# jfjell/Octree-Raymarcher

Measured on AMD Instinct MI355X. Metric: Mrays/s (primary+shadow) at 1920x1080, depth-12 SVO, higher is better.
Workload: dtype f32; 1 GPU; c3_1080p_depth12_4x1x4_shadow; depth_per_chunk=12, chunksize=128, nodes=99473656, bricks=34206642, hbm_pool_bytes=11087035656, kernel=auto, launches_in_flight=2, frames_per_launch=16, frames_in_flight=32, gather=False, partition=single, ranks_seen=1, launcher=single process

## Files before the change

octree-raymarcher_amd/csrc/kernel_stack.hip.h:

```cpp
#pragma once
#include "march.hip.h"
#include "step_asm.hip.h"
#include "chunk_step_asm.hip.h"

namespace svo {

constexpr int CW_ESCAPE_PENDING = (int)0x80000000;
enum : int { M_DONE = 0, M_WORLD = 1, M_HIT = 2, M_TREE = 3, M_TWIG = 4 };

constexpr int VOTE_WORLD = 8;
constexpr int VOTE_HIT = 16;
constexpr int VOTE_BUSY = 24;
constexpr int CREEP_SERIOUS = 6;
constexpr int CREEP_LANES = 8;
#define SVO_LIKELY(x) __builtin_expect(!!(x), 1)
#define SVO_UNLIKELY(x) __builtin_expect(!!(x), 0)
constexpr int STEP_EXTRA = 4;
constexpr int STEP_LANES = 8;
constexpr int DRAIN_STEPS = 8;
#ifndef SVO_SURE_MISS_WHEN
#define SVO_SURE_MISS_WHEN __builtin_amdgcn_readfirstlane(more ? 0 : 1)
#endif

__device__ __forceinline__ float recip_pow2(float x) { return __uint_as_float(0x7F000000u - __float_as_uint(x)); }

__device__ __forceinline__ unsigned long long vote(bool p) { return __builtin_amdgcn_ballot_w64(p); }
__device__ __forceinline__ int vote_count(unsigned long long m)
{
    int n = (int)__popcll(m);
    asm("" : "+s"(n));
    return n;
}

struct ChunkGrid {
    float inv;
    int32_t off[3];
    int32_t dimw, dimh, dimd;
    uint32_t table_in_lds;
};
static_assert(sizeof(ChunkGrid) == 32, "two 16-byte LDS reads");

__device__ __forceinline__ int wrap_once(int m, int dim)
{
    const uint32_t a = (uint32_t)m, b = (uint32_t)(m + dim), c = (uint32_t)(m - dim);
    return (int)min(min(a, b), c);
}

__device__ __forceinline__ void chunk_cell_pow2(const ChunkGrid &G, V3 p, int &mx, int &my, int &mz)
{
    float qx = p.x * G.inv, qy = p.y * G.inv, qz = p.z * G.inv;
    if (qx < 0.0f) qx -= 1.0f;
    if (qy < 0.0f) qy -= 1.0f;
    if (qz < 0.0f) qz -= 1.0f;
    const int ix = (int)qx, iy = (int)qy, iz = (int)qz;
    mx = wrap_once(ix + G.off[0], G.dimw); my = wrap_once(iy + G.off[1], G.dimh); mz = wrap_once(iz + G.off[2], G.dimd);
}
__device__ __forceinline__ uint32_t mad_u24(uint32_t a, uint32_t b, uint32_t c)
{
    uint32_t r;
    asm("v_mad_u32_u24 %0, %1, %2, %3" : "=v"(r) : "v"(a), "v"(b), "v"(c));
    return r;
}
__device__ __forceinline__ int chunk_index_u24(const ChunkGrid &G, int mx, int my, int mz)
{
    return (int)mad_u24(mad_u24((uint32_t)my, (uint32_t)G.dimd, (uint32_t)mz), (uint32_t)G.dimw, (uint32_t)mx);
}

__device__ __forceinline__ V3 cube_normal_pow2(V3 s, V3 lo, float size, float eps)
{
    const V3 hi = lo + size;
    const V3 c = (lo + hi) * 0.5f;
    const V3 p = s - c;
    const float d = fabsf(lo.x - hi.x) * 0.5f;
    const float invd = recip_pow2(d);
    const float b = 1.0f + eps;
    const float ix = (float)(int)((p.x * invd) * b), iy = (float)(int)((p.y * invd) * b), iz = (float)(int)((p.z * invd) * b);
    const float dot = ix * ix + iy * iy + iz * iz;
    float inv;
    if (dot == 1.0f) inv = 1.0f;
    else if (dot == 2.0f) inv = __uint_as_float(0x3F3504F3u);
    else if (dot == 3.0f) inv = __uint_as_float(0x3F13CD3Au);
    else inv = 1.0f / sqrtf(dot);
    return mk(ix * inv, iy * inv, iz * inv);
}

__device__ __forceinline__ uint32_t child_slot(int ux, int uy, int uz, int sh)
{
    const uint32_t bx = __builtin_amdgcn_ubfe((uint32_t)ux, (uint32_t)sh, 1u);
    const uint32_t by = __builtin_amdgcn_ubfe((uint32_t)uy, (uint32_t)sh, 1u);
    const uint32_t bz = __builtin_amdgcn_ubfe((uint32_t)uz, (uint32_t)sh, 1u);
    return ((bz << 1) + by) * 2u + bx;
}
__device__ __forceinline__ uint32_t ld_node(const uint32_t *pool, uint32_t boff)
{
    return *reinterpret_cast<const uint32_t *>(reinterpret_cast<const char *>(pool) + (size_t)boff);
}
constexpr uint32_t WIDE_PAYLOAD = (1u << 25) - 1u;
__device__ __forceinline__ uint32_t wide_slot(int ux, int uy, int uz, int sh)
{
    const uint32_t bx = __builtin_amdgcn_ubfe((uint32_t)ux, (uint32_t)sh, 2u);
    const uint32_t by = __builtin_amdgcn_ubfe((uint32_t)uy, (uint32_t)sh, 2u);
    const uint32_t bz = __builtin_amdgcn_ubfe((uint32_t)uz, (uint32_t)sh, 2u);
    return (bz << 4) | (by << 2) | bx;
}
__device__ __forceinline__ bool is_branch(uint32_t word) { return (int32_t)word < (int32_t)0xC0000000; }

__device__ __forceinline__ TraceArgs args_reloaded()
{
    auto p = __builtin_amdgcn_kernarg_segment_ptr();
    asm volatile("" : "+s"(p));
    TraceArgs T;
    __builtin_memcpy(&T, p, sizeof T);
    return T;
}
__device__ __forceinline__ FrameCam camera_reloaded(int f)
{
    auto p = __builtin_amdgcn_kernarg_segment_ptr();
    asm volatile("" : "+s"(p));
    FrameCam c;
    __builtin_memcpy(&c, (decltype(p))((const char __attribute__((address_space(4))) *)p + __builtin_offsetof(TraceArgs, cams) + (size_t)f * sizeof(FrameCam)), sizeof c);
    return c;
}

__device__ __noinline__ float brick_layer_first_touch(int k, V3 a, V3 b, V3 g, V3 bmin, float r, unsigned long long mask)
{
    const float ak = k == 0 ? a.x : k == 1 ? a.y : a.z, bk = k == 0 ? b.x : k == 1 ? b.y : b.z, mk_ = k == 0 ? bmin.x : k == 1 ? bmin.y : bmin.z;
    const float au = k == 0 ? a.y : k == 1 ? a.z : a.x, av = k == 0 ? a.z : k == 1 ? a.x : a.y;
    const float gu = k == 0 ? g.y : k == 1 ? g.z : g.x, gv = k == 0 ? g.z : k == 1 ? g.x : g.y;
    const float mu = k == 0 ? bmin.y : k == 1 ? bmin.z : bmin.x, mv = k == 0 ? bmin.z : k == 1 ? bmin.x : bmin.y;
    const int su = k == 0 ? 4 : k == 1 ? 16 : 1, sv = k == 0 ? 16 : k == 1 ? 1 : 4;
    const float delta = r * 0.0625f;
    bool ok = (ak == mk_) & (bk < 0.0f);
    ok &= (mu >= 4.0f * r) & (mv >= 4.0f * r) & (delta >= (fabsf(mu) + fabsf(mv) + 8.0f * r) * 0x1p-21f);
    ok = ok && fabsf(gu) < 1.0e30f && fabsf(gv) < 1.0e30f;
    if (!ok) return -1.0f;
    const float u0 = au - mu, v0 = av - mv;
    float first = __uint_as_float(0x7F800000u);
    bool clean = true;
    for (int cv = 0; cv < 4; ++cv) {
        const float va = ((float)cv * r - delta - v0) * gv, vb = ((float)(cv + 1) * r + delta - v0) * gv;
        const float v_in = fminf(va, vb), v_out = fmaxf(va, vb);
        for (int cu = 0; cu < 4; ++cu) {
            const bool occupied = (mask >> (cu * su + cv * sv)) & 1ull;
            const float ua = ((float)cu * r - delta - u0) * gu, ub = ((float)(cu + 1) * r + delta - u0) * gu;
            const float s_in = fmaxf(fmaxf(fminf(ua, ub), v_in), 0.0f), s_out = fminf(fmaxf(ua, ub), v_out);
            clean &= (s_in == s_in) & (s_out == s_out);
            first = (occupied & (s_in <= s_out)) ? fminf(first, s_in) : first;
        }
    }
    return clean ? first * (1.0f - 0x1p-18f) : -1.0f;
}

__device__ __forceinline__ void note_tile_cost(int outk, uint32_t steps)
{
    const TraceArgs T = args_reloaded();
    if (!T.tile_cost) return;
    const int k = outk & 0x7FFFFFFF;
    int tile, frame = 0;
    if (T.from_camera) {
        const int per = T.w * T.h;
        frame = k / per;
        const int r = k - frame * per;
        const int ly = r / T.w, lx = r - ly * T.w;
        tile = (ly / TILE_H) * T.tiles_per_row + lx / TILE_W;
    } else tile = k >> 6;
    atomicMax(&T.tile_cost[((size_t)frame * (size_t)T.ntiles + (size_t)tile) * 2 + (outk < 0 ? 1 : 0)], steps);
}

template <bool GLSL>
__device__ __forceinline__ bool past_far_end(int mode, float t, float tt_saved, float tw, float eps, float far)
{
    const float tt = mode == M_TWIG ? tt_saved : t;
    return (mode == M_TREE || mode == M_TWIG) && tw + (GLSL ? tt : tt - eps) >= far;
}

template <int MAXLV, int REFILL, int WAVES_PER_SIMD, bool BIG, bool GLSL, bool SEG = false>
__global__ __launch_bounds__(64, WAVES_PER_SIMD) void k_trace_stack(TraceArgs A)
{
    __shared__ uint32_t stk[MAXLV / 2 + 1][64];
    __shared__ float tile_ray[SEG ? 12 : 11][64];
    constexpr int CHUNK_TAB = (BIG && MAXLV <= 10) ? 126 : MAXLV > 16 ? 62 : 64;
    __shared__ uint32_t chunk_tab[6][CHUNK_TAB];
    __shared__ __attribute__((aligned(16))) ChunkGrid chunk_grid;
    stk[0][threadIdx.x] = 0u;
    const int lane = threadIdx.x;
    const bool want_cost = A.tile_cost != nullptr;
    [[maybe_unused]] const bool light_clear = (A.light_clear & LIGHT_CLEAR_NODES) != 0;
    const int n_chunks = A.dimw * A.dimh * A.dimd;
    const bool chunks_in_lds = n_chunks <= CHUNK_TAB;
    if (lane == 0) {
        chunk_grid.inv = A.inv_chunksize;
        for (int a = 0; a < 3; ++a) chunk_grid.off[a] = A.cbase[a] - A.ccm[a];
        chunk_grid.dimw = A.dimw; chunk_grid.dimh = A.dimh; chunk_grid.dimd = A.dimd;
        chunk_grid.table_in_lds = chunks_in_lds ? 1u : 0u;
    }
    if (chunks_in_lds)
        for (int i = lane; i < n_chunks; i += 64) {
            const DevWide ch = A.wchunks[i];
            chunk_tab[0][i] = __float_as_uint(ch.bmin[0]); chunk_tab[1][i] = __float_as_uint(ch.bmin[1]); chunk_tab[2][i] = __float_as_uint(ch.bmin[2]);
            chunk_tab[3][i] = ch.levels; chunk_tab[4][i] = ch.wide_off; chunk_tab[5][i] = (uint32_t)ch.twig_off;
        }
    __syncthreads();
#ifdef SVO_STACK_TIMING
    const unsigned long long t_begin = __builtin_amdgcn_s_memrealtime();
    unsigned n_iters = 0, n_tree_lanes = 0, n_twig_lanes = 0, n_world_lanes = 0;
    unsigned n_world_runs = 0, n_hit_runs = 0, n_refill = 0, n_tilegen = 0, n_fix = 0;
    unsigned n_lane_twig = 0;
    unsigned n_lane_busy = 0;
    unsigned n_creep_runs = 0, n_creep_rounds = 0, n_dbg = 0;
    unsigned n_wsteps = 0, n_lsteps = 0, n_hit_wait = 0, n_dead_wait = 0, n_wsteps_b = 0, n_lsteps_b = 0, n_world_wait = 0, n_twig_b = 0;
#endif
    [[maybe_unused]] StepStats step_stats;

    const V3 wlo = ld3(A.worldmin), whi = ld3(A.worldmax);
    const V3 sdir = ld3(A.sdir);
    const V3 sg = recip(sdir);
    const float eps = A.eps;
    const bool eps_pow2 = (__float_as_uint(eps) & 0x807FFFFFu) == 0u && __float_as_uint(eps) >= 0x00800000u && __float_as_uint(eps) < 0x7F800000u;
    const float csize = A.chunksize;

    const int tr_cols = A.tiles_per_row;
    const int tr_rows = A.ntiles / (tr_cols > 0 ? tr_cols : 1);
    const bool by_cols = tr_cols >= TILE_REGIONS;
    const int reg_q = (by_cols ? tr_cols : tr_rows) / TILE_REGIONS, reg_rem = (by_cols ? tr_cols : tr_rows) % TILE_REGIONS;
    int region = (int)(__builtin_amdgcn_s_getreg(20 | (0 << 6) | (3 << 11)) & (TILE_REGIONS - 1));
    int regions_left = TILE_REGIONS;
    int tile_first = 0;
    int tile_next = 64;
    bool more = true;
    unsigned rays_marched = 0;

    int mode = M_DONE;
    int outk = 0;
    V3 alpha = mk(0, 0, 0), beta = mk(0, 0, 1), g = mk(0, 0, 0);
    float tw = 0.0f;
    [[maybe_unused]] float far = __uint_as_float(0x7F800000u);
    int cw = 0;
    uint32_t guard = 0;
    V3 O = mk(0, 0, 0), Blo = mk(0, 0, 0);
    float res = 1.0f, t = 0.0f;
    int cnt = 0;
    float tt_saved = 0.0f, t_miss = 0.0f;
    int it_saved = 0;
    V3 clo = mk(0, 0, 0);
    WideRef<BIG> wide_b = 0;
    auto ld_wide = [&](uint32_t e) -> uint32_t {
        if constexpr (BIG) return *reinterpret_cast<const uint32_t *>((size_t)wide_b + ((size_t)e << 2));
        else return ld_node(A.wide, wide_b + (e << 2));
    };
    uint32_t twig_off = 0;
    int levels = 0, ci = -1;
    int pux = 0, puy = 0, puz = 0, valid = 0, plev = 0;
    unsigned long long bmask = 0;
#ifndef SVO_CXX_STEP
    float bsize = 0.0f, res_tree = 1.0f;
    int nw_chunk = 1;
    const uint32_t lds_lane = (uint32_t)(size_t)(__attribute__((address_space(3))) uint32_t *)&stk[0][lane];
    StepUniform SU;
    SU.csize = csize; SU.eps = eps; SU.eps2 = 2.0f * eps; SU.cap_twig = A.cap_twig; SU.wide = A.wide; SU.mask = A.mask; SU.descend_shift = MAXLV <= 10 ? DESCEND_SHIFT_SHALLOW : DESCEND_SHIFT_DEEP;
    const uint32_t lds_tab = (uint32_t)(size_t)(__attribute__((address_space(3))) uint32_t *)&chunk_tab[0][0];
    ChunkStepUniform CU;
    CU.wlo = wlo; CU.whi = whi; CU.csize = csize; CU.eps = eps; CU.cap_chunk = A.cap_chunk; CU.cap_tree = A.cap_tree; CU.wide = A.wide;
    CU.kernarg = __builtin_amdgcn_kernarg_segment_ptr();
#endif
    int creepn = 0;
    for (;;) {
        unsigned long long dead = vote(mode == M_DONE);
        while (more && vote_count(dead) >= REFILL) {
            if (tile_next >= 64) {
                int t32 = -1, tcol = 0, trow = 0, tframe = 0;
                const uint32_t *order = args_reloaded().tile_order;
                if (order) {
                    regions_left = 0;
                    unsigned long long tix = 0;
                    if (lane == 0) tix = atomicAdd(&A.work[WORK_CURSOR0], 1ull);
                    int t = __builtin_amdgcn_readfirstlane((int)tix);
                    if (t < A.ntiles * A.nframes) {
                        tframe = t / A.ntiles; t -= tframe * A.ntiles;
                        t32 = (int)order[t];
                        if ((uint32_t)t32 >= (uint32_t)A.ntiles) { t32 = 0; tframe = -1; }
                        trow = t32 / tr_cols; tcol = t32 - trow * tr_cols;
                    }
                }
                while (regions_left > 0) {
                    const int span = reg_q + (region < reg_rem ? 1 : 0);
                    const int first = region * reg_q + (region < reg_rem ? region : reg_rem);
                    const int count = span * (by_cols ? tr_rows : tr_cols);
                    unsigned long long tix = 0;
                    if (lane == 0) tix = atomicAdd(&A.work[WORK_CURSOR0 + region], 1ull);
                    int t = __builtin_amdgcn_readfirstlane((int)tix);
                    if (t < count * A.nframes) {
                        if (A.nframes > 1) { tframe = t / count; t -= tframe * count; }
                        if (by_cols) { trow = t / span; tcol = first + (t - trow * span); }
                        else { trow = first + t / tr_cols; tcol = t % tr_cols; }
                        t32 = trow * tr_cols + tcol;
                        break;
                    }
                    region = (region + 1) & (TILE_REGIONS - 1);
                    --regions_left;
                }
                if (t32 < 0) { more = false; break; }
                tile_first = t32 * 64;
                tile_next = 0;
#ifdef SVO_STACK_TIMING
                ++n_tilegen;
#endif
                {
                    const TraceArgs T = args_reloaded();
                    const int id = tile_first + lane;
                    bool ok;
                    int k = -1;
                    V3 o = mk(0, 0, 0), d = mk(0, 0, 1);
                    if (T.from_camera) {
                        const int lx = tcol * TILE_W + (lane & (TILE_W - 1));
                        const int ly = trow * TILE_H + lane / TILE_W;
                        ok = (lx < T.w) & (ly < T.h) & (tframe >= 0);
                        k = (tframe * T.h + ly) * T.w + lx;
                        int px = 0, py = 0;
                        if (ok) local_to_pixel(T, lx, ly, px, py);
                        if (ok && (py >= T.imgh || px >= T.imgw)) { store_miss(A.out, k, 0); ok = false; }
                        if (ok) camera_ray(camera_reloaded(tframe), T.imgw, T.imgh, px, py, o, d);
                    } else {
                        ok = id < T.n && tframe >= 0;
                        k = id;
                        if (ok) { o = ld3(T.origins + 3 * (long long)id); d = ld3(T.dirs + 3 * (long long)id); }
                        if constexpr (SEG) tile_ray[11][lane] = ok ? T.tmax[id] : 0.0f;
                    }
                    const V3 gg = recip(d);
                    float t0 = 0.0f;
                    if (ok) {
                        bool hit = true;
                        if (!inside(o, wlo, whi)) t0 = (GLSL ? enter_glsl(o, gg, wlo, whi, hit) : enter(o, d, wlo, whi, hit)) + eps;
                        rays_marched++;
                        if (!hit) { store_miss(A.out, k, 0); ok = false; }
                    }
                    tile_ray[0][lane] = o.x; tile_ray[1][lane] = o.y; tile_ray[2][lane] = o.z;
                    tile_ray[3][lane] = d.x; tile_ray[4][lane] = d.y; tile_ray[5][lane] = d.z;
                    tile_ray[6][lane] = gg.x; tile_ray[7][lane] = gg.y; tile_ray[8][lane] = gg.z;
                    tile_ray[9][lane] = t0;
                    tile_ray[10][lane] = __int_as_float(ok ? k : -1);
                    __syncthreads();
                }
            }
#ifdef SVO_STACK_TIMING
            ++n_refill;
#endif
            const int rank = (int)__builtin_amdgcn_mbcnt_hi((unsigned)(dead >> 32), __builtin_amdgcn_mbcnt_lo((unsigned)dead, 0u));
            const int avail = 64 - tile_next;
            if (mode == M_DONE && rank < avail) {
                const int slot = tile_next + rank;
                const int k = __float_as_int(tile_ray[10][slot]);
                if (k >= 0) {
                    outk = k;
                    alpha = mk(tile_ray[0][slot], tile_ray[1][slot], tile_ray[2][slot]);
                    beta = mk(tile_ray[3][slot], tile_ray[4][slot], tile_ray[5][slot]);
                    g = mk(tile_ray[6][slot], tile_ray[7][slot], tile_ray[8][slot]);
                    tw = tile_ray[9][slot];
                    if constexpr (SEG) far = tile_ray[11][slot];
                    cw = 0; guard = 0; creepn = 0;
                    mode = M_WORLD;
                }
            }
            const int ndead = vote_count(dead);
            tile_next += (ndead < avail) ? ndead : avail;
            __syncthreads();
            dead = vote(mode == M_DONE);
        }
        if (dead == ~0ull) break;
#ifdef SVO_STACK_TIMING
        ++n_iters;
        n_tree_lanes += __popcll(__ballot(mode == M_TREE)); n_twig_lanes += __popcll(__ballot(mode == M_TWIG));
        n_world_lanes += __popcll(__ballot(mode == M_WORLD));
#endif

        const int n_busy = vote_count(vote(mode == M_TREE || mode == M_TWIG));
        const int n_world = vote_count(vote(mode == M_WORLD));
        const int n_hit = vote_count(vote(mode == M_HIT));
        const bool few_busy = n_busy < VOTE_BUSY;
        bool run_world = n_world >= (few_busy ? 1 : VOTE_WORLD);
        if (!run_world && n_world > 0) run_world = vote(mode == M_WORLD && creepn <= -CREEP_SERIOUS) != 0ull;
        const bool run_hit = n_hit >= (few_busy ? 1 : VOTE_HIT);

        if (SVO_UNLIKELY(mode != M_DONE && mode != M_HIT && ++guard > STEP_GUARD)) {
            if (outk < 0) store_flags(A.out, outk & 0x7FFFFFFF, SVO_HIT_FLAG | SVO_SHADOW_TRACED | SVO_ERR_FLAG | (A.normal_mode == SVO_NORMAL_FACE ? (uint32_t)SVO_FACE_NORMAL : 0u));
            else store_miss(A.out, outk, SVO_ERR_FLAG);
            mode = M_DONE;
        }

#ifdef SVO_STACK_TIMING
        n_world_runs += run_world; n_hit_runs += run_hit;
#endif
        if (SVO_LIKELY(run_world)) { asm volatile("");
#ifndef SVO_CXX_STEP
        const ChunkGrid G = chunk_grid;
        const unsigned long long missed = ChunkStepAsm<BIG, GLSL, SEG>::template run<CHUNK_TAB>(
            mode, tw, cw, ci, valid, pux, puy, puz, clo, wide_b, twig_off, levels, O, t, cnt, Blo, res, bsize, res_tree, nw_chunk,
            alpha, beta, g, far, G.inv, G.off[0], G.off[1], G.off[2], G.dimw, G.dimh, G.dimd,
            (uint32_t)__builtin_amdgcn_readfirstlane((int)G.table_in_lds), lds_tab, CU);
        if (__builtin_amdgcn_inverse_ballot_w64(missed)) {
            int k = outk;
            asm("" : "+v"(k));
            if (k >= 0) store_miss(A.out, k, 0);
            if (want_cost) note_tile_cost(k, guard);
            mode = M_DONE;
        }
#else
        if (mode == M_WORLD) {
            if (cw < 0) {
                cw &= ~CW_ESCAPE_PENDING;
                if constexpr (GLSL) tw += guarded(escape(O, g, clo, clo + csize), eps) + eps;
                else tw += escape(O, g, clo, clo + csize) + eps;
            }
            bool miss = cw >= A.cap_chunk;
            if constexpr (SEG) miss |= (GLSL ? tw : tw - eps) >= far;
            if (!miss) {
                cw++;
// ... 44 lines not shown
        }

        int pass = 0;
        const int fixed_steps = (n_busy >= STEP_LANES && vote(creepn > 0 || creepn <= -4 * CREEP_SERIOUS) == 0ull) ? STEP_EXTRA : 0;
#ifndef SVO_CXX_STEP
        const unsigned long long shadow_lanes = light_clear ? vote(outk < 0) : 0ull;
#endif
        for (;;) {
#ifdef SVO_STACK_TIMING
        n_lane_twig += mode == M_TWIG ? (pass == 0 ? 1u + (unsigned)fixed_steps : (unsigned)DRAIN_STEPS) : 0u;
        n_lane_busy += (mode == M_TREE || mode == M_TWIG) ? (pass == 0 ? 1u + (unsigned)fixed_steps : (unsigned)DRAIN_STEPS) : 0u;
        { const int nm = __popcll(__ballot(mode == M_TREE || mode == M_TWIG)); n_wsteps += nm > 0; n_lsteps += nm; if (more) { n_wsteps_b += nm > 0; n_lsteps_b += nm; n_hit_wait += __popcll(__ballot(mode == M_HIT)); n_dead_wait += __popcll(__ballot(mode == M_DONE)); n_world_wait += __popcll(__ballot(mode == M_WORLD)); n_twig_b += __popcll(__ballot(mode == M_TWIG)); } }
#endif
#ifndef SVO_CXX_STEP
        const int nsteps = pass == 0 ? 1 + fixed_steps : DRAIN_STEPS;
        const int sure_miss = SVO_SURE_MISS_WHEN;
        march_steps_asm<BIG, GLSL>(mode, O, Blo, bsize, res, t, cnt, tt_saved, t_miss, it_saved, tw, cw, pux, puy, puz, valid, plev, bmask, creepn,
                                   beta, g, clo, alpha, levels, nw_chunk, res_tree, wide_b, twig_off, lds_lane, SU, nsteps | (sure_miss << 16), shadow_lanes, step_stats);
        pass += nsteps - 1;
#else
        if (mode == M_TREE || mode == M_TWIG) {
            enum : int { S_LEAVE = 0, S_ADVANCE = 1, S_ENTER = 2, S_HIT_LEAF = 3, S_HIT_CELL = 4, S_BAD = 5 };
            const bool twig = mode == M_TWIG;
            const float Bsize = twig ? res * 4.0f : csize, inv_res = recip_pow2(res);
            const int crept = creepn < 0 ? -creepn : creepn;
            creepn = -crept;
            bool leave = cnt <= 0;
            cnt -= 1;
            const V3 p = O + beta * t;
            leave |= !inside(p, Blo, Blo + Bsize);
            const float fx = (p.x - Blo.x) * inv_res, fy = (p.y - Blo.y) * inv_res, fz = (p.z - Blo.z) * inv_res;
            int ux = (int)fx, uy = (int)fy, uz = (int)fz;
#ifdef SVO_STACK_TIMING
            n_fix += __ballot(!twig && ((fx == (float)ux) | (fy == (float)uy) | (fz == (float)uz))) != 0;
#endif
            if (SVO_UNLIKELY(!twig && ((fx == (float)ux) | (fy == (float)uy) | (fz == (float)uz)))) {
                const int nmax = (1 << levels) - 1;
                ux = ux > nmax ? nmax : ux; uy = uy > nmax ? nmax : uy; uz = uz > nmax ? nmax : uz;
                ux -= (Blo.x + (float)ux * res > p.x) ? 1 : 0;
                uy -= (Blo.y + (float)uy * res > p.y) ? 1 : 0;
                uz -= (Blo.z + (float)uz * res > p.z) ? 1 : 0;
            }
            if (twig) leave |= (ux > 3) | (uy > 3) | (uz > 3);

            int what = S_LEAVE;
            int low = 0;
            uint32_t payload = 0;
            if (SVO_LIKELY(!leave)) {
                if (!twig) {
                    const uint32_t diff = (uint32_t)((ux ^ pux) | (uy ^ puy) | (uz ^ puz));
                    const int nw = levels ? (levels + 1) >> 1 : 1;
                    const int hb = 32 - __clz((int)(diff | 1u));
                    const int keep = nw - ((hb + 1) >> 1);
                    int k;
                    asm("v_med3_i32 %0, %1, 0, %2" : "=v"(k) : "v"(keep), "v"(valid));
                    uint32_t wnode = stk[k][lane];
                    int sh = 2 * (nw - 1 - k);
                    uint32_t word = ld_wide((wnode << 6) + wide_slot(ux, uy, uz, sh));
                    while (is_branch(word)) {
                        wnode = word & WIDE_PAYLOAD;
                        ++k;
                        stk[k][lane] = wnode;
                        sh -= 2;
                        word = ld_wide((wnode << 6) + wide_slot(ux, uy, uz, sh));
                    }
                    valid = k; pux = ux; puy = uy; puz = uz;
                    plev = (int)((word >> 25) & 31u);
                    low = (1 << (levels - plev)) - 1;
                    const uint32_t type = node_type(word);
                    what = type == EMPTY ? S_ADVANCE : type == LEAF ? S_HIT_LEAF : S_ENTER;
                    payload = word;
                } else {
                    payload = (uint32_t)(uz * 16 + uy * 4 + ux);
                    what = ((bmask >> payload) & 1ull) ? S_HIT_CELL : S_ADVANCE;
                }
            }

            if (what == S_ADVANCE || what == S_ENTER) {
                const V3 E_lo = mk(Blo.x + (float)(ux & ~low) * res, Blo.y + (float)(uy & ~low) * res, Blo.z + (float)(uz & ~low) * res);
                const float E_size = res * (float)(low + 1);
                const float e = (GLSL ? guarded(escape(p, g, E_lo, E_lo + E_size), eps) : escape(p, g, E_lo, E_lo + E_size)) + eps;
                if (what == S_ADVANCE) {
                    t += e;
                    creepn = e < 2.0f * eps ? crept + 1 : 0;
                } else {
                    bmask = A.mask[twig_off + (payload & WIDE_PAYLOAD)];
                    tt_saved = t; t_miss = t + e; it_saved = cnt;
                    O = p; t = 0.0f; cnt = A.cap_twig;
                    Blo = E_lo;
                    res = E_size * 0.25f;
                    mode = M_TWIG;
                }
            }
            if (leave) {
                if (twig) {
                    t = t_miss;
                    cnt = it_saved;
                    O = alpha + beta * tw;
                    Blo = clo;
                    res = csize * __uint_as_float((uint32_t)(127 - levels) << 23);
                    mode = M_TREE;
                } else {
                    cw |= CW_ESCAPE_PENDING;
                    mode = M_WORLD;
                }
            }
            if (what == S_HIT_LEAF) {
                tw = tw + (GLSL ? t : t - eps);
                cnt = (int)SVO_CELL_NONE;
                mode = M_HIT;
            }
            if (what == S_HIT_CELL) {
                float sdist = t;
                sdist += tt_saved;
                tw = tw + sdist;
                cnt = (int)payload;
                mode = M_HIT;
            }
        }
#endif

        ++pass;
        if (pass <= fixed_steps) continue;
        if (more || pass >= 256) break;
        const unsigned long long marching = vote(mode == M_TREE || mode == M_TWIG);
        if (marching == 0ull || marching != vote(mode != M_DONE) || vote(creepn > 0 || creepn <= -4 * CREEP_SERIOUS) != 0ull) break;
        if constexpr (SEG) if (vote(past_far_end<GLSL>(mode, t, tt_saved, tw, eps, far)) != 0ull) break;
        }
        guard += pass - 1;
        if constexpr (SEG) {
            if (past_far_end<GLSL>(mode, t, tt_saved, tw, eps, far)) {
                if (mode == M_TWIG) O = alpha + beta * tw;
                creepn = creepn > 0 ? -creepn : creepn;
                cw |= CW_ESCAPE_PENDING;
                mode = M_WORLD;
            }
        }

#include "creep_block.inc"

        if (mode == M_HIT && outk < 0) {
            store_flags(A.out, outk & 0x7FFFFFFF, SVO_HIT_FLAG | SVO_SHADOW_TRACED | SVO_SHADOWED | (A.normal_mode == SVO_NORMAL_FACE ? (uint32_t)SVO_FACE_NORMAL : 0u));
            if (want_cost) note_tile_cost(outk, guard);
            mode = M_DONE;
        }
        if constexpr (SEG) {
            if (mode == M_HIT && !(tw < far)) {
                store_miss(A.out, outk, 0);
                if (want_cost) note_tile_cost(outk, guard);
                mode = M_DONE;
            }
        }
        if (run_hit) { asm volatile("");
        if (mode == M_HIT) {
            const int nw = levels ? (levels + 1) >> 1 : 1;
            const uint32_t wn = valid > 0 ? stk[valid][lane] : 0u, slot = wide_slot(pux, puy, puz, 2 * (nw - 1 - valid));
            const uint32_t word = ld_wide((wn << 6) + slot);
            uint32_t node = 0u;
            if (plev != 0) {
                const uint32_t ci = ((slot >> 1) & 1u) | ((slot >> 2) & 2u) | ((slot >> 3) & 4u);
                const uint32_t gi = (slot & 1u) | ((slot >> 1) & 2u) | ((slot >> 2) & 4u);
                size_t wnode_in_pool;
                if constexpr (BIG) wnode_in_pool = (((size_t)wide_b - (size_t)A.wide) >> 8) + wn;
                else wnode_in_pool = (wide_b >> 8) + wn;
                const uint32_t *wb = A.wbase + wnode_in_pool * WIDE_BASE_WORDS;
                const int level_child = 2 * valid + 1 - (2 * nw - levels);
                const bool child = plev == level_child;
                node = wb[child ? 0u : 1u + ci] + (child ? ci : gi);
            }
            const uint32_t hitc = (uint32_t)cnt;
            V3 vlo;
            float vsize;
            uint32_t material;
            if (hitc == SVO_CELL_NONE) {
                const int low = (1 << (levels - plev)) - 1;
                vlo = mk(Blo.x + (float)(pux & ~low) * res, Blo.y + (float)(puy & ~low) * res, Blo.z + (float)(puz & ~low) * res);
                vsize = res * (float)(low + 1);
                material = word & 0xFFFFu;
            } else {
                vlo = mk(Blo.x + (float)(hitc & 3u) * res, Blo.y + (float)((hitc >> 2) & 3u) * res, Blo.z + (float)(hitc >> 4) * res);
                vsize = res;
                const unsigned long long brick = (unsigned long long)twig_off + (word & WIDE_PAYLOAD);
                const uint32_t bw = A.bmat[brick];
                material = bw == BMAT_SEVERAL ? A.twig[brick * TWIG_WORDS + hitc] : (bw & BMAT_MATERIAL_MASK) | ((bw & BMAT_CLEAR_BIT) << 1);
            }
            const V3 point = alpha + beta * (tw - eps);
            uint32_t dark = 0u;
            if constexpr (!GLSL && !SEG) {
                const uint32_t use = (uint32_t)A.light_clear & (uint32_t)(LIGHT_CLEAR_BRICKS | LIGHT_CLEAR_DARK);
                if (use != 0u) {
                    const float inv_res = recip_pow2(res);
                    const float dx = point.x - Blo.x, dy = point.y - Blo.y, dz = point.z - Blo.z;
                    const uint32_t ux = (uint32_t)(int)(dx * inv_res), uy = (uint32_t)(int)(dy * inv_res), uz = (uint32_t)(int)(dz * inv_res);
                    const bool located = (hitc != SVO_CELL_NONE) & (dx >= 0.0f) & (dy >= 0.0f) & (dz >= 0.0f) & ((ux | uy | uz) <= 3u);
                    const uint32_t occupied = (uint32_t)(bmask >> ((uz * 16u + uy * 4u + ux) & 63u)) & 1u;
                    const uint32_t on = (use >> (1u + occupied)) & (occupied | (material >> 16)) & 1u;
                    const uint32_t settle = located ? on : 0u;
                    material = (material & 0xFFFFu) | (settle << 16);
                    dark = (settle & occupied) * (uint32_t)SVO_SHADOWED;
                } else {
                    material &= 0xFFFFu;
                }
            }
            const bool face = A.normal_mode == SVO_NORMAL_FACE;
            const V3 n = face ? face_normal(point, vlo, vlo + vsize, beta) : cube_normal_pow2(point, vlo, vsize, eps);
            const uint32_t flags = SVO_HIT_FLAG | (A.shadow ? SVO_SHADOW_TRACED : 0u) | (face ? (uint32_t)SVO_FACE_NORMAL : 0u) | dark;
            store_hit(A.out, outk, tw, n, material, flags, (uint32_t)ci, node, hitc);
            if (want_cost) note_tile_cost(outk, guard);
            mode = M_DONE;
            if (A.shadow) {
                alpha = point; beta = sdir; g = sg;
                outk |= (int)0x80000000;
                if constexpr (SEG) far = __uint_as_float(0x7F800000u);
                tw = 0.0f; cw = 0; guard = 0; creepn = 0;
                bool hit = true;
                if (!inside(alpha, wlo, whi)) tw = (GLSL ? enter_glsl(alpha, g, wlo, whi, hit) : enter(alpha, beta, wlo, whi, hit)) + eps;
                const bool settled = !GLSL && !SEG && (material >> 16) != 0u;
                mode = hit && !settled ? M_WORLD : M_DONE;
                rays_marched++;
            }
        } }
    }

    unsigned total = rays_marched;
    for (int off = 32; off > 0; off >>= 1) total += __shfl_down(total, off, 64);
    if (lane == 0 && total) atomicAdd(&A.work[1], (unsigned long long)total);
#ifdef SVO_STACK_TIMING
    unsigned busiest = n_lane_busy;
    for (int off = 32; off > 0; off >>= 1) busiest = max(busiest, (unsigned)__shfl_xor((int)busiest, off, 64));
    unsigned busiest_twig = n_lane_busy == busiest ? n_lane_twig : 0u;
    for (int off = 32; off > 0; off >>= 1) busiest_twig = max(busiest_twig, (unsigned)__shfl_xor((int)busiest_twig, off, 64));
    if (lane == 0 && A.counters) {
        uint4 c; c.x = (uint32_t)t_begin; c.y = (uint32_t)__builtin_amdgcn_s_memrealtime(); c.z = n_iters; c.w = total;
        reinterpret_cast<uint4 *>(A.counters)[6 * blockIdx.x] = c;
        uint4 e; e.x = n_world_runs | (n_hit_runs << 16); e.y = n_refill | (n_tilegen << 12) | (n_fix << 20); e.z = n_tree_lanes; e.w = n_twig_lanes | (n_world_lanes << 20);
        reinterpret_cast<uint4 *>(A.counters)[6 * blockIdx.x + 1] = e;
        uint4 f; f.x = n_creep_runs | (busiest_twig << 16); f.y = busiest; f.z = n_creep_rounds; f.w = n_dbg;
        reinterpret_cast<uint4 *>(A.counters)[6 * blockIdx.x + 2] = f;
        uint4 h; h.x = n_wsteps; h.y = n_lsteps; h.z = n_hit_wait; h.w = n_dead_wait;
        reinterpret_cast<uint4 *>(A.counters)[6 * blockIdx.x + 3] = h;
        uint4 h2; h2.x = n_wsteps_b; h2.y = n_lsteps_b; h2.z = n_world_wait; h2.w = n_twig_b;
        reinterpret_cast<uint4 *>(A.counters)[6 * blockIdx.x + 4] = h2;
        uint4 h3; h3.x = step_stats.steps; h3.y = step_stats.lanes; h3.z = step_stats.stalls; h3.w = step_stats.chased;
        reinterpret_cast<uint4 *>(A.counters)[6 * blockIdx.x + 5] = h3;
    }
#endif
}

}
```

Baseline: 9190 Mrays/s.

## Replace C++ hit-resolve block with hand-written inline assembly

Moves the hit-resolution path (wide-node lookup, voxel bounds, normal computation, hit store and shadow-ray setup) into a hand-scheduled inline-asm routine specialised per BIG/GLSL/SEG variant. The aim is to cut instruction count, control scalar/vector register use, overlap the dependent global loads with the normal math, and control exec masking directly. The out-of-bounds enter() and cost accounting remain in C++. It adds a large maintenance burden and risks subtle correctness issues, such as hazard nops, hard-coded clobbered registers and the different settle logic.

```diff
diff --git a/octree-raymarcher_amd/csrc/hit_resolve_asm.hip.h b/octree-raymarcher_amd/csrc/hit_resolve_asm.hip.h
--- /dev/null
+++ b/octree-raymarcher_amd/csrc/hit_resolve_asm.hip.h
@@ -0,0 +1,50 @@
+#pragma once
+#include "march.hip.h"
+#include "chunk_step_asm.hip.h"
+
+namespace svo {
+
+struct HitResolveUniform {
+    V3 wlo, whi, sdir;
+    float eps;
+    const uint32_t *wide, *wbase;
+    const uint16_t *twig;
+    void *out;
+    uint32_t use;
+    uint32_t fb16;
+    decltype(__builtin_amdgcn_kernarg_segment_ptr()) kernarg;
+};
+
+template <bool BIG, bool GLSL, bool SEG>
+struct HitResolveAsm;
+
+#define SVO_HIT_BIG false
+#define SVO_HIT_GLSL false
+#define SVO_HIT_SEG false
+#include "hit_resolve_body.inc"
+#undef SVO_HIT_SEG
+#define SVO_HIT_SEG true
+#include "hit_resolve_body.inc"
+#undef SVO_HIT_GLSL
+#define SVO_HIT_GLSL true
+#include "hit_resolve_body.inc"
+#undef SVO_HIT_SEG
+#define SVO_HIT_SEG false
+#include "hit_resolve_body.inc"
+#undef SVO_HIT_BIG
+#define SVO_HIT_BIG true
+#include "hit_resolve_body.inc"
+#undef SVO_HIT_SEG
+#define SVO_HIT_SEG true
+#include "hit_resolve_body.inc"
+#undef SVO_HIT_GLSL
+#define SVO_HIT_GLSL false
+#include "hit_resolve_body.inc"
+#undef SVO_HIT_SEG
+#define SVO_HIT_SEG false
+#include "hit_resolve_body.inc"
+#undef SVO_HIT_BIG
+#undef SVO_HIT_GLSL
+#undef SVO_HIT_SEG
+
+}
diff --git a/octree-raymarcher_amd/csrc/hit_resolve_body.inc b/octree-raymarcher_amd/csrc/hit_resolve_body.inc
--- /dev/null
+++ b/octree-raymarcher_amd/csrc/hit_resolve_body.inc
@@ -0,0 +1,381 @@
+#if !SVO_HIT_GLSL && !SVO_HIT_SEG
+#define SVO_HIT_SETTLE 1
+#else
+#define SVO_HIT_SETTLE 0
+#endif
+
+template <>
+struct HitResolveAsm<SVO_HIT_BIG, SVO_HIT_GLSL, SVO_HIT_SEG> {
+static __device__ __forceinline__ unsigned long long run(
+    int &mode, int &outk, V3 &alpha, V3 &beta, V3 &g, float &tw, int &cw, uint32_t &guard, int &creepn, [[maybe_unused]] float &far,
+    unsigned &rays_marched, unsigned long long &outside, uint32_t &steps,
+    const int valid, const int plev, const int levels, const int nw, const int pux, const int puy, const int puz, const int cnt, const int ci,
+    const WideRef<SVO_HIT_BIG> wide_b, const uint32_t twig_off, const V3 Blo, const float res, [[maybe_unused]] const unsigned long long bmask,
+    const uint32_t lds_lane, const V3 sg, const HitResolveUniform U)
+{
+    uint32_t q0, q1, q2, q3, q4, q5, q6;
+    unsigned long long sall, shit, sout, ss1, ss2, ss3, sbm;
+    asm volatile(
+        "s_mov_b64 %[sall], exec\n\t"
+        "s_mov_b64 %[sout], 0\n\t"
+        "v_cmpx_eq_u32 vcc, 2, %[md]\n\t"
+        "s_mov_b64 %[shit], exec\n\t"
+        "s_cbranch_execz 9f\n\t"
+        "s_load_dwordx2 %[sbm], %[karg], %[bmatoff]\n\t"
+        "v_max_i32 %[q0], 0, %[val]\n\t"
+        "v_lshl_add_u32 %[q0], %[q0], 8, %[ldsl]\n\t"
+        "ds_read_b32 v0, %[q0]\n\t"
+        "v_not_b32 %[q1], %[val]\n\t"
+        "v_add_lshl_u32 %[q1], %[nw], %[q1], 1\n\t"
+        "v_bfe_u32 %[q2], %[pux], %[q1], 2\n\t"
+        "v_bfe_u32 %[q3], %[puy], %[q1], 2\n\t"
+        "v_bfe_u32 %[q1], %[puz], %[q1], 2\n\t"
+        "v_lshlrev_b32 %[q1], 4, %[q1]\n\t"
+        "v_lshl_or_b32 %[q1], %[q3], 2, %[q1]\n\t"
+        "v_or_b32 %[q1], %[q1], %[q2]\n\t"
+        "v_bfe_u32 %[q4], %[q1], 1, 1\n\t"
+        "v_lshrrev_b32 %[q3], 2, %[q1]\n\t"
+        "v_lshrrev_b32 %[q5], 3, %[q1]\n\t"
+        "v_and_b32 %[q6], 2, %[q3]\n\t"
+        "v_and_b32 %[q5], 4, %[q5]\n\t"
+        "v_or3_b32 %[q4], %[q4], %[q6], %[q5]\n\t"
+        "v_and_b32 %[q2], 1, %[q2]\n\t"
+        "v_lshrrev_b32 %[q5], 1, %[q1]\n\t"
+        "v_and_b32 %[q5], 2, %[q5]\n\t"
+        "v_and_b32 %[q3], 4, %[q3]\n\t"
+        "v_or3_b32 %[q2], %[q5], %[q2], %[q3]\n\t"
+        "v_lshlrev_b32 %[q3], 1, %[nw]\n\t"
+        "v_sub_u32 %[q3], %[lev], %[q3]\n\t"
+        "v_lshl_add_u32 %[q3], %[val], 1, %[q3]\n\t"
+        "v_add_u32 %[q3], 1, %[q3]\n\t"
+        "v_cmp_eq_u32 vcc, %[plv], %[q3]\n\t"
+        "v_add_u32 %[q3], 1, %[q4]\n\t"
+        "v_lshlrev_b32 %[q5], 2, %[q1]\n\t"
+        "v_cndmask_b32 %[q2], %[q2], %[q4], vcc\n\t"
+        "v_cndmask_b32_e64 %[q3], %[q3], 0, vcc\n\t"
+        "s_waitcnt lgkmcnt(0)\n\t"
+#if SVO_HIT_BIG
+        "v_lshl_add_u32 %[q5], v0, 6, %[q1]\n\t"
+        "v_mad_u64_u32 v[2:3], vcc, %[q5], 4, %[wb]\n\t"
+        "global_load_dword v5, v[2:3], off\n\t"
+        "v_lshl_add_u64 v[8:9], %[wb], 0, 0\n\t"
+        "v_subrev_co_u32 v8, vcc, %[widelo], v8\n\t"
+        "v_mov_b32 %[q4], %[widehi]\n\t"
+        "s_nop 0\n\t"
+        "v_subb_co_u32 v9, vcc, v9, %[q4], vcc\n\t"
+        "v_alignbit_b32 %[q0], v9, v8, 8\n\t"
+        "v_add_u32 %[q0], v0, %[q0]\n\t"
+#else
+        "v_lshl_add_u32 %[q5], v0, 8, %[q5]\n\t"
+        "v_add_u32 %[q5], %[wb], %[q5]\n\t"
+        "global_load_dword v5, %[q5], %[wide]\n\t"
+        "v_lshrrev_b32 %[q0], 8, %[wb]\n\t"
+        "v_add_u32 %[q0], v0, %[q0]\n\t"
+#endif
+        "v_mad_u64_u32 v[8:9], vcc, %[q0], 36, %[wbase]\n\t"
+        "v_mad_u64_u32 v[8:9], vcc, %[q3], 4, v[8:9]\n\t"
+        "global_load_dword v6, v[8:9], off\n\t"
+        "v_subrev_f32 %[q0], %[eps], %[tw]\n\t"
+        "v_mul_f32 %[q1], %[bx], %[q0]\n\t"
+        "v_mul_f32 %[q3], %[by], %[q0]\n\t"
+        "v_mul_f32 %[q0], %[bz], %[q0]\n\t"
+        "v_add_f32 %[ax], %[ax], %[q1]\n\t"
+        "v_add_f32 %[ay], %[ay], %[q3]\n\t"
+        "v_add_f32 %[az], %[az], %[q0]\n\t"
+        "v_sub_u32 %[q0], %[lev], %[plv]\n\t"
+        "v_lshlrev_b32_e64 %[q0], %[q0], 1\n\t"
+        "v_sub_u32 %[q1], 0, %[q0]\n\t"
+        "v_and_b32 %[q3], %[pux], %[q1]\n\t"
+        "v_and_b32 %[q4], %[puy], %[q1]\n\t"
+        "v_and_b32 %[q5], %[puz], %[q1]\n\t"
+        "v_cvt_f32_i32 %[q0], %[q0]\n\t"
+        "v_cmpx_ne_u32 vcc, 0xff, %[cnt]\n\t"
+        "s_mov_b64 %[ss1], exec\n\t"
+        "s_cbranch_execz 1f\n\t"
+        "v_and_b32 %[q3], 3, %[cnt]\n\t"
+        "v_bfe_u32 %[q4], %[cnt], 2, 2\n\t"
+        "v_lshrrev_b32 %[q5], 4, %[cnt]\n\t"
+        "v_mov_b32 %[q0], 1.0\n\t"
+        "s_waitcnt vmcnt(1)\n\t"
+        "v_and_b32 %[q1], 0x1ffffff, v5\n\t"
+        "v_mad_u64_u32 v[8:9], vcc, %[tof], 2, %[sbm]\n\t"
+        "v_mad_u64_u32 v[8:9], vcc, %[q1], 2, v[8:9]\n\t"
+        "global_load_ushort v7, v[8:9], off\n\t"
+        "1:\n\t"
+        "s_mov_b64 exec, %[shit]\n\t"
+        "v_cvt_f32_i32 %[q3], %[q3]\n\t"
+        "v_cvt_f32_i32 %[q4], %[q4]\n\t"
+        "v_cvt_f32_i32 %[q5], %[q5]\n\t"
+        "v_mul_f32 %[q0], %[rs], %[q0]\n\t"
+        "v_mul_f32 %[q3], %[rs], %[q3]\n\t"
+        "v_mul_f32 %[q4], %[rs], %[q4]\n\t"
+        "v_mul_f32 %[q5], %[rs], %[q5]\n\t"
+        "v_add_f32 %[q3], %[lx], %[q3]\n\t"
+        "v_add_f32 %[q4], %[ly], %[q4]\n\t"
+        "v_add_f32 %[q5], %[lz], %[q5]\n\t"
+        "v_add_f32 %[q1], %[q0], %[q3]\n\t"
+        "v_add_f32 %[q6], %[q0], %[q4]\n\t"
+        "v_add_f32 %[q0], %[q0], %[q5]\n\t"
+        "v_sub_f32 v0, %[q3], %[q1]\n\t"
+        "v_add_f32 %[q1], %[q3], %[q1]\n\t"
+        "v_add_f32 %[q6], %[q4], %[q6]\n\t"
+        "v_add_f32 %[q0], %[q5], %[q0]\n\t"
+        "v_mul_f32 %[q1], 0.5, %[q1]\n\t"
+        "v_mul_f32 %[q6], 0.5, %[q6]\n\t"
+        "v_mul_f32 %[q0], 0.5, %[q0]\n\t"
+        "v_sub_f32 %[q3], %[ax], %[q1]\n\t"
+        "v_sub_f32 %[q4], %[ay], %[q6]\n\t"
+        "v_sub_f32 %[q5], %[az], %[q0]\n\t"
+        "s_bitcmp1_b32 %[fb], %[facebit]\n\t"
+        "s_cbranch_scc1 3f\n\t"
+        "v_mul_f32_e64 v0, |v0|, 0.5\n\t"
+        "v_sub_u32 v0, 0x7f000000, v0\n\t"
+        "v_add_f32 %[q1], 1.0, %[eps]\n\t"
+        "v_mul_f32 %[q3], %[q3], v0\n\t"
+        "v_mul_f32 %[q4], %[q4], v0\n\t"
+        "v_mul_f32 %[q5], %[q5], v0\n\t"
+        "v_mul_f32 %[q3], %[q1], %[q3]\n\t"
+        "v_mul_f32 %[q4], %[q1], %[q4]\n\t"
+        "v_mul_f32 %[q5], %[q1], %[q5]\n\t"
+        "v_cvt_i32_f32 %[q3], %[q3]\n\t"
+        "v_cvt_i32_f32 %[q4], %[q4]\n\t"
+        "v_cvt_i32_f32 %[q5], %[q5]\n\t"
+        "v_cvt_f32_i32 %[q3], %[q3]\n\t"
+        "v_cvt_f32_i32 %[q4], %[q4]\n\t"
+        "v_cvt_f32_i32 %[q5], %[q5]\n\t"
+        "v_mul_f32 %[q0], %[q3], %[q3]\n\t"
+        "v_mul_f32 %[q6], %[q4], %[q4]\n\t"
+        "v_add_f32 %[q0], %[q0], %[q6]\n\t"
+        "v_mul_f32 %[q6], %[q5], %[q5]\n\t"
+        "v_add_f32 %[q0], %[q6], %[q0]\n\t"
+        "v_cmp_eq_f32 vcc, 2.0, %[q0]\n\t"
+        "v_cmp_eq_f32_e64 %[ss2], 1.0, %[q0]\n\t"
+        "v_mov_b32 %[q6], 0x3f3504f3\n\t"
+        "v_mov_b32 v0, 0x3f13cd3a\n\t"
+        "v_cndmask_b32_e64 %[q1], 1.0, %[q6], vcc\n\t"
+        "s_or_b64 %[ss2], %[ss2], vcc\n\t"
+        "v_cmp_eq_f32 vcc, 0x40400000, %[q0]\n\t"
+        "s_or_b64 %[ss2], %[ss2], vcc\n\t"
+        "s_andn2_b64 %[ss2], exec, %[ss2]\n\t"
+        "v_cndmask_b32 %[q1], %[q1], v0, vcc\n\t"
+        "s_cbranch_scc1 4f\n\t"
+        "40:\n\t"
+        "v_mul_f32 v1, %[q1], %[q3]\n\t"
+        "v_mul_f32 v2, %[q1], %[q4]\n\t"
+        "v_mul_f32 v3, %[q1], %[q5]\n\t"
+        "30:\n\t"
+#if SVO_HIT_SETTLE
+        "s_cmp_lg_u32 %[use], 0\n\t"
+        "s_cbranch_scc0 6f\n\t"
+        "v_sub_u32 %[q0], 0x7f000000, %[rs]\n\t"
+        "v_sub_f32 %[q1], %[ax], %[lx]\n\t"
+        "v_sub_f32 %[q3], %[ay], %[ly]\n\t"
+        "v_sub_f32 %[q4], %[az], %[lz]\n\t"
+        "v_mul_f32 %[q5], %[q1], %[q0]\n\t"
+        "v_mul_f32 %[q6], %[q3], %[q0]\n\t"
+        "v_mul_f32 %[q0], %[q4], %[q0]\n\t"
+        "v_cvt_i32_f32 %[q5], %[q5]\n\t"
+        "v_cvt_i32_f32 %[q6], %[q6]\n\t"
+        "v_cvt_i32_f32 %[q0], %[q0]\n\t"
+        "s_mov_b64 exec, %[ss1]\n\t"
+        "v_cmpx_le_f32 vcc, 0, %[q1]\n\t"
+        "v_cmpx_le_f32 vcc, 0, %[q3]\n\t"
+        "v_cmpx_le_f32 vcc, 0, %[q4]\n\t"
+        "v_or3_b32 %[q1], %[q5], %[q6], %[q0]\n\t"
+        "v_cmpx_gt_u32 vcc, 4, %[q1]\n\t"
+        "s_mov_b64 %[ss2], exec\n\t"
+        "s_mov_b64 exec, %[shit]\n\t"
+        "v_lshlrev_b32 %[q0], 4, %[q0]\n\t"
+        "v_lshlrev_b32 %[q6], 2, %[q6]\n\t"
+        "v_add3_u32 %[q0], %[q6], %[q5], %[q0]\n\t"
+        "v_lshrrev_b64 v[8:9], %[q0], %[bm]\n\t"
+        "v_and_b32 %[q0], 1, v8\n\t"
+        "v_add_u32 %[q1], 1, %[q0]\n\t"
+        "v_lshrrev_b32_e64 %[q1], %[q1], %[use]\n\t"
+        "60:\n\t"
+#endif
+        "s_waitcnt vmcnt(0)\n\t"
+        "v_and_b32 %[q3], 0x7fff, v7\n\t"
+        "v_and_b32 %[q4], 0x8000, v7\n\t"
+        "v_cmp_eq_u32 vcc, 0xffff, v7\n\t"
+        "v_lshl_or_b32 %[q3], %[q4], 1, %[q3]\n\t"
+        "v_and_b32 %[q4], 0xffff, v5\n\t"
+        "s_and_b64 vcc, vcc, %[ss1]\n\t"
+        "s_cbranch_scc1 5f\n\t"
+        "50:\n\t"
+        "v_cndmask_b32_e64 %[q4], %[q4], %[q3], %[ss1]\n\t"
+        "v_add_u32 v6, v6, %[q2]\n\t"
+        "v_cmp_ne_u32 vcc, 0, %[plv]\n\t"
+        "v_mov_b32 v0, %[tw]\n\t"
+        "v_mov_b32 v5, %[ci]\n\t"
+        "v_cndmask_b32_e64 v6, 0, v6, vcc\n\t"
+        "v_mov_b32 v7, %[cnt]\n\t"
+        "v_and_b32 v4, 0xffff, %[q4]\n\t"
+        "v_or_b32 v4, %[fb], v4\n\t"
+#if SVO_HIT_SETTLE
+        "v_lshrrev_b32 %[q3], 16, %[q4]\n\t"
+        "v_or_b32 %[q3], %[q0], %[q3]\n\t"
+        "v_and_b32 %[q1], %[q1], %[q3]\n\t"
+        "v_and_b32 %[q1], 1, %[q1]\n\t"
+        "v_cndmask_b32_e64 %[q1], 0, %[q1], %[ss2]\n\t"
+        "v_and_b32 %[q0], %[q1], %[q0]\n\t"
+        "v_lshl_or_b32 v4, %[q0], %[darksh], v4\n\t"
+#endif
+        "v_mad_u64_u32 v[8:9], vcc, %[outk], 32, %[out]\n\t"
+        "v_mov_b32 %[q2], %[gd]\n\t"
+        "global_store_dwordx4 v[8:9], v[0:3], off\n\t"
+        "global_store_dwordx4 v[8:9], v[4:7], off offset:16\n\t"
+        "s_bitcmp1_b32 %[fb], %[shadowbit]\n\t"
+        "s_cbranch_scc0 8f\n\t"
+        "v_mov_b32 %[bx], %[sdx]\n\t"
+        "v_mov_b32 %[by], %[sdy]\n\t"
+        "v_mov_b32 %[bz], %[sdz]\n\t"
+        "v_mov_b32 %[gx], %[sgx]\n\t"
+        "v_mov_b32 %[gy], %[sgy]\n\t"
+        "v_mov_b32 %[gz], %[sgz]\n\t"
+        "v_or_b32 %[outk], 0x80000000, %[outk]\n\t"
+#if SVO_HIT_SEG
+        "v_mov_b32 %[far], 0x7f800000\n\t"
+#endif
+#if SVO_HIT_SETTLE
+        "v_cmp_eq_u32 vcc, 0, %[q1]\n\t"
+#endif
+        "v_mov_b32 %[tw], 0\n\t"
+        "v_mov_b32 %[cw], 0\n\t"
+        "v_mov_b32 %[gd], 0\n\t"
+        "v_mov_b32 %[crn], 0\n\t"
+        "v_add_u32 %[rm], 1, %[rm]\n\t"
+#if SVO_HIT_SETTLE
+        "v_cndmask_b32_e64 %[md], 0, 1, vcc\n\t"
+        "s_and_b64 exec, exec, vcc\n\t"
+#else
+        "v_mov_b32 %[md], 1\n\t"
+#endif
+        "s_mov_b64 %[ss1], exec\n\t"
+        "v_cmpx_le_f32 vcc, %[wlx], %[ax]\n\t"
+        "v_cmpx_le_f32 vcc, %[wly], %[ay]\n\t"
+        "v_cmpx_le_f32 vcc, %[wlz], %[az]\n\t"
+        "v_cmpx_ge_f32 vcc, %[whx], %[ax]\n\t"
+        "v_cmpx_ge_f32 vcc, %[why], %[ay]\n\t"
+        "v_cmpx_ge_f32 vcc, %[whz], %[az]\n\t"
+        "s_andn2_b64 %[sout], %[ss1], exec\n\t"
+        "s_branch 9f\n\t"
+        "8:\n\t"
+        "v_mov_b32 %[md], 0\n\t"
+        "s_branch 9f\n\t"
+        "3:\n\t"
+        "v_cmp_gt_f32_e64 %[ss2], |%[q4]|, |%[q3]|\n\t"
+        "v_and_b32 %[q0], 0x7fffffff, %[q3]\n\t"
+        "v_and_b32 %[q1], 0x7fffffff, %[q4]\n\t"
+        "v_cndmask_b32_e64 %[q0], %[q0], %[q1], %[ss2]\n\t"
+        "v_cndmask_b32_e64 %[q1], %[q3], %[q4], %[ss2]\n\t"
+        "v_cndmask_b32_e64 %[q6], %[bx], %[by], %[ss2]\n\t"
+        "v_cmp_gt_f32_e64 %[ss3], |%[q5]|, %[q0]\n\t"
+        "s_andn2_b64 %[ss2], %[ss2], %[ss3]\n\t"
+        "s_nop 0\n\t"
+        "v_cndmask_b32_e64 %[q1], %[q1], %[q5], %[ss3]\n\t"
+        "v_cndmask_b32_e64 %[q6], %[q6], %[bz], %[ss3]\n\t"
+        "s_nop 0\n\t"
+        "v_cmp_lt_f32 vcc, 0, %[q6]\n\t"
+        "s_nop 1\n\t"
+        "v_cndmask_b32_e64 %[q6], 1.0, -1.0, vcc\n\t"
+        "v_cmp_gt_f32 vcc, 0, %[q1]\n\t"
+        "s_nop 1\n\t"
+        "v_cndmask_b32_e64 %[q6], %[q6], -1.0, vcc\n\t"
+        "v_cmp_lt_f32 vcc, 0, %[q1]\n\t"
+        "s_nop 1\n\t"
+        "v_cndmask_b32_e64 %[q6], %[q6], 1.0, vcc\n\t"
+        "s_or_b64 vcc, %[ss2], %[ss3]\n\t"
+        "v_cndmask_b32_e64 v2, 0, %[q6], %[ss2]\n\t"
+        "v_cndmask_b32_e64 v3, 0, %[q6], %[ss3]\n\t"
+        "v_cndmask_b32_e64 v1, %[q6], 0, vcc\n\t"
+        "s_branch 30b\n\t"
+        "4:\n\t"
+        "s_mov_b64 exec, %[ss2]\n\t"
+        "v_mul_f32 %[q1], 0x4f800000, %[q0]\n\t"
+        "v_cmp_gt_f32 vcc, 0xf800000, %[q0]\n\t"
+        "s_nop 1\n\t"
+        "v_cndmask_b32 %[q1], %[q0], %[q1], vcc\n\t"
+        "v_sqrt_f32 %[q6], %[q1]\n\t"
+        "s_nop 0\n\t"
+        "v_add_u32 v0, -1, %[q6]\n\t"
+        "v_fma_f32 v8, -v0, %[q6], %[q1]\n\t"
+        "v_add_u32 v4, 1, %[q6]\n\t"
+        "v_cmp_ge_f32_e64 %[ss3], 0, v8\n\t"
+        "s_nop 1\n\t"
+        "v_cndmask_b32_e64 v0, %[q6], v0, %[ss3]\n\t"
+        "v_fma_f32 %[q6], -v4, %[q6], %[q1]\n\t"
+        "v_cmp_lt_f32_e64 %[ss3], 0, %[q6]\n\t"
+        "s_nop 1\n\t"
+        "v_cndmask_b32_e64 %[q6], v0, v4, %[ss3]\n\t"
+        "v_mul_f32 v0, 0x37800000, %[q6]\n\t"
+        "v_cndmask_b32 %[q6], %[q6], v0, vcc\n\t"
+        "v_mov_b32 v0, 0x260\n\t"
+        "v_cmp_class_f32 vcc, %[q1], v0\n\t"
+        "s_nop 1\n\t"
+        "v_cndmask_b32 %[q1], %[q6], %[q1], vcc\n\t"
+        "v_div_scale_f32 %[q6], %[ss3], %[q1], %[q1], 1.0\n\t"
+        "v_rcp_f32 v0, %[q6]\n\t"
+        "s_nop 0\n\t"
+        "v_fma_f32 v4, -%[q6], v0, 1.0\n\t"
+        "v_fmac_f32 v0, v4, v0\n\t"
+        "v_div_scale_f32 v4, vcc, 1.0, %[q1], 1.0\n\t"
+        "v_mul_f32 v8, v4, v0\n\t"
+        "v_fma_f32 v9, -%[q6], v8, v4\n\t"
+        "v_fmac_f32 v8, v9, v0\n\t"
+        "v_fma_f32 %[q6], -%[q6], v8, v4\n\t"
+        "v_div_fmas_f32 %[q6], %[q6], v0, v8\n\t"
+        "v_div_fixup_f32 %[q1], %[q6], %[q1], 1.0\n\t"
+        "s_mov_b64 exec, %[shit]\n\t"
+        "s_branch 40b\n\t"
+        "5:\n\t"
+        "s_mov_b64 exec, vcc\n\t"
+        "v_and_b32 %[q5], 0x1ffffff, v5\n\t"
+        "v_mov_b32 %[q6], 0x80\n\t"
+        "v_mad_u64_u32 v[8:9], vcc, %[tof], %[q6], %[twig]\n\t"
+        "v_mad_u64_u32 v[8:9], vcc, %[q5], %[q6], v[8:9]\n\t"
+        "v_mad_u64_u32 v[8:9], vcc, %[cnt], 2, v[8:9]\n\t"
+        "global_load_ushort %[q3], v[8:9], off\n\t"
+        "s_mov_b64 exec, %[shit]\n\t"
+        "s_waitcnt vmcnt(0)\n\t"
+        "s_branch 50b\n\t"
+#if SVO_HIT_SETTLE
+        "6:\n\t"
+        "s_mov_b64 %[ss2], 0\n\t"
+        "v_mov_b32 %[q0], 0\n\t"
+        "v_mov_b32 %[q1], 0\n\t"
+        "s_branch 60b\n\t"
+#endif
+        "9:\n\t"
+        "s_mov_b64 exec, %[sall]\n\t"
+        : [md] "+v"(mode), [outk] "+v"(outk), [ax] "+v"(alpha.x), [ay] "+v"(alpha.y), [az] "+v"(alpha.z),
+          [bx] "+v"(beta.x), [by] "+v"(beta.y), [bz] "+v"(beta.z), [gx] "+v"(g.x), [gy] "+v"(g.y), [gz] "+v"(g.z),
+          [tw] "+v"(tw), [cw] "+v"(cw), [gd] "+v"(guard), [crn] "+v"(creepn), [rm] "+v"(rays_marched),
+#if SVO_HIT_SEG
+          [far] "+v"(far),
+#endif
+          [q0] "=&v"(q0), [q1] "=&v"(q1), [q2] "=&v"(q2), [q3] "=&v"(q3), [q4] "=&v"(q4), [q5] "=&v"(q5), [q6] "=&v"(q6),
+          [sall] "=&s"(sall), [shit] "=&s"(shit), [sout] "=&s"(sout), [ss1] "=&s"(ss1), [ss2] "=&s"(ss2), [ss3] "=&s"(ss3), [sbm] "=&s"(sbm)
+        : [val] "v"(valid), [plv] "v"(plev), [lev] "v"(levels), [nw] "v"(nw), [pux] "v"(pux), [puy] "v"(puy), [puz] "v"(puz),
+          [cnt] "v"(cnt), [ci] "v"(ci), [wb] "v"(wide_b), [tof] "v"(twig_off), [lx] "v"(Blo.x), [ly] "v"(Blo.y), [lz] "v"(Blo.z), [rs] "v"(res),
+          [ldsl] "v"(lds_lane), [sgx] "v"(sg.x), [sgy] "v"(sg.y), [sgz] "v"(sg.z),
+#if SVO_HIT_SETTLE
+          [bm] "v"(bmask), [use] "s"(U.use), [darksh] "n"(16 + __builtin_ctz((unsigned)SVO_SHADOWED)),
+#endif
+#if SVO_HIT_BIG
+          [widelo] "s"((uint32_t)(size_t)U.wide), [widehi] "s"((uint32_t)((size_t)U.wide >> 32)),
+#else
+          [wide] "s"(U.wide),
+#endif
+          [wbase] "s"(U.wbase), [twig] "s"(U.twig), [out] "s"(U.out), [fb] "s"(U.fb16), [eps] "s"(U.eps),
+          [sdx] "s"(U.sdir.x), [sdy] "s"(U.sdir.y), [sdz] "s"(U.sdir.z),
+          [wlx] "s"(U.wlo.x), [wly] "s"(U.wlo.y), [wlz] "s"(U.wlo.z), [whx] "s"(U.whi.x), [why] "s"(U.whi.y), [whz] "s"(U.whi.z),
+          [karg] "s"(U.kernarg), [bmatoff] "n"(__builtin_offsetof(TraceArgs, bmat)),
+          [facebit] "n"(16 + __builtin_ctz((unsigned)SVO_FACE_NORMAL)), [shadowbit] "n"(16 + __builtin_ctz((unsigned)SVO_SHADOW_TRACED))
+        : "v0", "v1", "v2", "v3", "v4", "v5", "v6", "v7", "v8", "v9", "vcc", "scc", "memory");
+    outside = sout;
+    steps = q2;
+    return shit;
+}
+};
+#undef SVO_HIT_SETTLE
diff --git a/octree-raymarcher_amd/csrc/kernel_stack.hip.h b/octree-raymarcher_amd/csrc/kernel_stack.hip.h
--- a/octree-raymarcher_amd/csrc/kernel_stack.hip.h
+++ b/octree-raymarcher_amd/csrc/kernel_stack.hip.h
@@ -2,6 +2,7 @@
 #include "march.hip.h"
 #include "step_asm.hip.h"
 #include "chunk_step_asm.hip.h"
+#include "hit_resolve_asm.hip.h"
 
 namespace svo {
 
@@ -244,7 +245,7 @@
     int it_saved = 0;
     V3 clo = mk(0, 0, 0);
     WideRef<BIG> wide_b = 0;
-    auto ld_wide = [&](uint32_t e) -> uint32_t {
+    [[maybe_unused]] auto ld_wide = [&](uint32_t e) -> uint32_t {
         if constexpr (BIG) return *reinterpret_cast<const uint32_t *>((size_t)wide_b + ((size_t)e << 2));
         else return ld_node(A.wide, wide_b + (e << 2));
     };
@@ -262,6 +263,13 @@
     ChunkStepUniform CU;
     CU.wlo = wlo; CU.whi = whi; CU.csize = csize; CU.eps = eps; CU.cap_chunk = A.cap_chunk; CU.cap_tree = A.cap_tree; CU.wide = A.wide;
     CU.kernarg = __builtin_amdgcn_kernarg_segment_ptr();
+#ifndef SVO_CXX_HIT
+    HitResolveUniform HU;
+    HU.wlo = wlo; HU.whi = whi; HU.sdir = sdir; HU.eps = eps; HU.wide = A.wide; HU.wbase = A.wbase; HU.twig = A.twig; HU.out = A.out;
+    HU.use = (!GLSL && !SEG) ? (uint32_t)A.light_clear & (uint32_t)(LIGHT_CLEAR_BRICKS | LIGHT_CLEAR_DARK) : 0u;
+    HU.fb16 = (SVO_HIT_FLAG | (A.shadow ? (uint32_t)SVO_SHADOW_TRACED : 0u) | (A.normal_mode == SVO_NORMAL_FACE ? (uint32_t)SVO_FACE_NORMAL : 0u)) << 16;
+    HU.kernarg = CU.kernarg;
+#endif
 #endif
     int creepn = 0;
     for (;;) {
@@ -612,6 +620,21 @@
             }
         }
         if (run_hit) { asm volatile("");
+#if !defined(SVO_CXX_STEP) && !defined(SVO_CXX_HIT)
+        unsigned long long outside;
+        uint32_t steps;
+        const unsigned long long resolved = HitResolveAsm<BIG, GLSL, SEG>::run(
+            mode, outk, alpha, beta, g, tw, cw, guard, creepn, far, rays_marched, outside, steps,
+            valid, plev, levels, nw_chunk, pux, puy, puz, cnt, ci, wide_b, twig_off, Blo, res, bmask, lds_lane, sg, HU);
+        if (want_cost) {
+            if (__builtin_amdgcn_inverse_ballot_w64(resolved)) note_tile_cost(outk & 0x7FFFFFFF, steps);
+        }
+        if (__builtin_amdgcn_inverse_ballot_w64(outside)) {
+            bool hit = true;
+            tw = (GLSL ? enter_glsl(alpha, g, wlo, whi, hit) : enter(alpha, beta, wlo, whi, hit)) + eps;
+            if (!hit) mode = M_DONE;
+        }
+#else
         if (mode == M_HIT) {
             const int nw = levels ? (levels + 1) >> 1 : 1;
             const uint32_t wn = valid > 0 ? stk[valid][lane] : 0u, slot = wide_slot(pux, puy, puz, 2 * (nw - 1 - valid));
@@ -679,7 +702,9 @@
                 mode = hit && !settled ? M_WORLD : M_DONE;
                 rays_marched++;
             }
-        } }
+        }
+#endif
+        }
     }
 
     unsigned total = rays_marched;
```

Result: no change. 9273 Mrays/s (median of 6 runs) (+0.9%).
